# apache/tez

Hardware: NVIDIA H100
Metric: sorted KV GB/s (16B key / 64B val) (higher is better)
Workload: dtype u8

## Files before the change

### tez_b200/csrc/emit_fast.cuh

```cuda
#pragma once
#include "sorter_kernels.cuh"

#ifndef TEZGPU_EMIT_MIN_CTAS
#define TEZGPU_EMIT_MIN_CTAS 4
#endif

namespace tezgpu {

constexpr int FE_THREADS = 256;
constexpr int FE_MAX_RECS = 256;
constexpr int FE_IMG_BYTES = 22016;

struct TileDesc {
  uint32_t p;
  uint32_t r0;
  uint32_t nr;
  uint32_t flags;
  uint64_t abs0;
  uint64_t after;
};

struct TileCrc {
  uint32_t raw;
  uint32_t p;
// ... 6 lines not shown
  int lo = 0, hi = e.P;
  while (hi - lo > 1) {
    int mid = (lo + hi) >> 1;
    if (e.tile_start[mid] <= tile) lo = mid; else hi = mid;
  }
  const uint32_t p = (uint32_t)lo;
  const uint32_t ps = e.part_start[p], pe = e.part_start[p + 1];
  const uint32_t k = tile - e.tile_start[p];
  TileDesc d;
  d.p = p;
  d.r0 = ps + k * e.recs_per_tile;
  d.nr = min(e.recs_per_tile, pe - d.r0);
  const bool first = (k == 0), last = (d.r0 + d.nr == pe);
  d.flags = (first ? 1u : 0u) | (last ? 2u : 0u);
  const uint64_t seg0 = e.seg_start[p];
  d.abs0 = seg0 + (first ? 0 : 4 + (uint64_t)(d.r0 - ps) * e.rec_size);
  const uint64_t tile_end = seg0 + 4 + (uint64_t)(d.r0 - ps + d.nr) * e.rec_size + (last ? 2 : 0);
  d.after = (e.seg_start[p + 1] - 4) - tile_end;
  tiles[tile] = d;
}

__global__ void k_crc_combine(const TileCrc *__restrict__ tc, uint32_t ntiles, const CrcTables *__restrict__ t,
                              uint32_t *__restrict__ seg_crc) {
  uint32_t i = blockIdx.x * blockDim.x + threadIdx.x;
  const int lane = threadIdx.x & 31;
  uint32_t p = 0xFFFFFFFFu, val = 0;
  if (i < ntiles) {
    TileCrc c = tc[i];
    p = c.p;
    val = c.raw ? crc_shift_bytes(t, c.raw, c.after) : 0u;
  }
#pragma unroll
  for (int o = 1; o < 32; o <<= 1) {
    uint32_t v2 = __shfl_up_sync(0xffffffffu, val, o), p2 = __shfl_up_sync(0xffffffffu, p, o);
    if (lane >= o && p2 == p) val ^= v2;
  }
  uint32_t pn = __shfl_down_sync(0xffffffffu, p, 1);
  if (p != 0xFFFFFFFFu && (lane == 31 || pn != p) && val) atomicXor(&seg_crc[p], val);
}

__device__ __forceinline__ void sts_b8(uint32_t a, uint32_t v) { asm volatile("st.shared.b8 [%0], %1;" ::"r"(a), "r"(v) : "memory"); }
__device__ __forceinline__ void sts_b16(uint32_t a, uint32_t v) { asm volatile("st.shared.b16 [%0], %1;" ::"r"(a), "h"((unsigned short)v) : "memory"); }
__device__ __forceinline__ void sts_b32(uint32_t a, uint32_t v) { asm volatile("st.shared.b32 [%0], %1;" ::"r"(a), "r"(v) : "memory"); }
__device__ __forceinline__ void sts_v4(uint32_t a, uint4 v) {
  asm volatile("st.shared.v4.b32 [%0], {%1,%2,%3,%4};" ::"r"(a), "r"(v.x), "r"(v.y), "r"(v.z), "r"(v.w) : "memory");
}

__device__ __forceinline__ void sts16_unaligned(uint32_t a, uint4 v) {
  const uint32_t al = a & 3u;
  if (al == 0) {
    if ((a & 15u) == 0) sts_v4(a, v);
    else { sts_b32(a, v.x); sts_b32(a + 4, v.y); sts_b32(a + 8, v.z); sts_b32(a + 12, v.w); }
  } else if (al == 2) {
    sts_b16(a, v.x & 0xFFFFu);
    sts_b32(a + 2, __funnelshift_r(v.x, v.y, 16));
    sts_b32(a + 6, __funnelshift_r(v.y, v.z, 16));
    sts_b32(a + 10, __funnelshift_r(v.z, v.w, 16));
    sts_b16(a + 14, v.w >> 16);
  } else if (al == 1) {
    sts_b8(a, v.x & 0xFFu);
    sts_b16(a + 1, (v.x >> 8) & 0xFFFFu);
    sts_b32(a + 3, __funnelshift_r(v.x, v.y, 24));
    sts_b32(a + 7, __funnelshift_r(v.y, v.z, 24));
    sts_b32(a + 11, __funnelshift_r(v.z, v.w, 24));
    sts_b8(a + 15, v.w >> 24);
  } else {
    sts_b8(a, v.x & 0xFFu);
    sts_b32(a + 1, __funnelshift_r(v.x, v.y, 8));
    sts_b32(a + 5, __funnelshift_r(v.y, v.z, 8));
    sts_b32(a + 9, __funnelshift_r(v.z, v.w, 8));
    sts_b16(a + 13, (v.w >> 8) & 0xFFFFu);
    sts_b8(a + 15, v.w >> 24);
  }
}

__device__ __forceinline__ uint4 ldg_stream_v4(const void *p) {
  uint4 r;
  asm volatile("ld.global.nc.L1::no_allocate.v4.u32 {%0,%1,%2,%3}, [%4];"
               : "=r"(r.x), "=r"(r.y), "=r"(r.z), "=r"(r.w) : "l"(p));
  return r;
}
__device__ __forceinline__ void stg_stream_v4(void *p, uint4 v) {
  asm volatile("st.global.L1::no_allocate.v4.u32 [%0], {%1,%2,%3,%4};" ::"l"(p), "r"(v.x), "r"(v.y), "r"(v.z), "r"(v.w) : "memory");
}

struct FastEmitParams {
  EmitParams e;
  const TileDesc *tiles;
  TileCrc *tile_crc;
  uint32_t ntiles;
  uint32_t cpr;
  uint32_t cpr_magic;
  uint32_t stride;
};

__device__ __forceinline__ uint64_t fast_source_offset(const Records &rec, uint32_t ri, uint32_t stride, uint32_t p) {
  if (rec.use_runs) return run_record_off_p(rec.runs, p, ri) + rec.runs.hdr_len;
  return rec.key_off ? rec.key_off[ri] : (uint64_t)ri * stride;
}

template <int UNROLL, bool ALIGNED>
__global__ void __launch_bounds__(FE_THREADS, TEZGPU_EMIT_MIN_CTAS) k_emit_fast(FastEmitParams fp) {
  __shared__ __align__(16) uint8_t s_img[FE_IMG_BYTES];
  __shared__ uint32_t s_idx[2][FE_MAX_RECS];
  __shared__ uint64_t s_off[ALIGNED ? 1 : 2][ALIGNED ? 1 : FE_MAX_RECS];
  __shared__ uint32_t s_tab[4 * 256];
  __shared__ uint32_t s_adv32[4 * 256];
  __shared__ uint32_t s_part[FE_THREADS];

  const EmitParams &e = fp.e;
  const int tid = threadIdx.x, lane = tid & 31, warp = tid >> 5;
  for (int i = tid; i < 4 * 256; i += FE_THREADS) {
    s_tab[i] = (&e.crc->slice[0][0])[i];
    s_adv32[i] = (&e.crc->adv128[0][0])[i];
  }
  const uint32_t lane_pow = e.crc->pow_word[4 * (31 - lane)];
  WarpLinearMap m_word, m_skip;
  {
    const uint32_t *gt = &e.crc->slice[0][0], *ga = &e.crc->advc[0][0];
    m_word.init([&](uint32_t x) { return gt[768 + (x & 0xFF)] ^ gt[512 + ((x >> 8) & 0xFF)] ^ gt[256 + ((x >> 16) & 0xFF)] ^ gt[x >> 24]; }, lane);
    m_skip.init([&](uint32_t x) { return ga[x & 0xFF] ^ ga[256 + ((x >> 8) & 0xFF)] ^ ga[512 + ((x >> 16) & 0xFF)] ^ ga[768 + (x >> 24)]; }, lane);
  }
  const uint32_t img_base = (uint32_t)__cvta_generic_to_shared(s_img);
  const uint8_t *__restrict__ kv = e.rec.kv;
  const uint8_t *kv_end = kv + e.rec.kv_bytes;
  const uint32_t rec_size = e.rec_size, hdr_len = e.fixed_hdr_len, stride = fp.stride;

  TileDesc td_next;
  if (blockIdx.x < fp.ntiles) {
    td_next = fp.tiles[blockIdx.x];
    if ((uint32_t)tid < td_next.nr) {
      const uint32_t ri = e.order[td_next.r0 + tid];
      s_idx[0][tid] = ri;
      if (!ALIGNED) s_off[0][tid] = fast_source_offset(e.rec, ri, stride, td_next.p);
    }
  }
  uint32_t buf = 0;
  for (uint32_t tile = blockIdx.x; tile < fp.ntiles; tile += gridDim.x, buf ^= 1u) {
    const TileDesc td = td_next;
    const uint32_t nr = td.nr;
    const bool first_tile = td.flags & 1u, last_tile = td.flags & 2u;
    const uint32_t tile_n = tile + gridDim.x;
    if (tile_n < fp.ntiles) td_next = fp.tiles[tile_n];
    __syncthreads();
    const uint32_t *__restrict__ c_idx = s_idx[buf];
    const uint64_t *__restrict__ c_off = s_off[ALIGNED ? 0 : buf];
    const uint64_t abs0 = td.abs0;
    const uint32_t lead = (uint32_t)(abs0 & 15u);
    const uint32_t rec0 = lead + (first_tile ? 4u : 0u);
    const uint32_t body_end = rec0 + nr * rec_size + (last_tile ? 2u : 0u);

    const uint32_t npieces = nr * fp.cpr;
    const uint32_t half_up = (nr + 1) >> 1;
    for (uint32_t q0 = tid; q0 < npieces; q0 += FE_THREADS * UNROLL) {
      uint4 v[UNROLL];
      uint32_t dst[UNROLL];
#pragma unroll
      for (int u = 0; u < UNROLL; u++) {
        uint32_t q = q0 + u * FE_THREADS;
        if (q < npieces) {
          uint32_t jp = fp.cpr == 1 ? q : __umulhi(q, fp.cpr_magic);
          uint32_t c = q - jp * fp.cpr;
          uint32_t j = jp < half_up ? 2u * jp : 2u * (jp - half_up) + 1u;
          if (ALIGNED) {
            v[u] = ldg_stream_v4(kv + (uint64_t)c_idx[j] * stride + 16u * c);
          } else {
// ... 112 lines not shown
```

### tez_b200/csrc/emit_pipe.cuh

```cuda
#pragma once
#include "emit_fast.cuh"

#ifndef TEZGPU_EMIT4_MIN_CTAS
#define TEZGPU_EMIT4_MIN_CTAS 3
#endif

namespace tezgpu {

constexpr int FE4_BATCH = FE_THREADS / 32;
constexpr int FE4_UNROLL = 5;
constexpr int FE4_RUN = 5;
constexpr uint32_t FE4_RUN_BYTES = 16u * FE4_RUN;
constexpr int FE4_IMG_BYTES = FE_THREADS * FE4_RUN * 16;
constexpr int FE4_GROUPS = 2;
constexpr int FE4_PARKED = 4;
constexpr int FE4_WBITS = 7;
constexpr int FE4_WDIGITS = (32 + FE4_WBITS - 1) / FE4_WBITS;
constexpr int FE4_WENTRIES = ((FE4_WDIGITS - 1) << FE4_WBITS) + (1 << (32 - FE4_WBITS * (FE4_WDIGITS - 1)));

static inline uint32_t emit4_max_recs(uint32_t rec_size) {
  return std::min<uint32_t>(FE_MAX_RECS, (FE4_IMG_BYTES - 15 - 4 - 2) / rec_size);
}

constexpr uint32_t FE4_MAX_CPR = 8;

static inline bool emit4_fits(uint32_t recs, uint32_t cpr, uint32_t rec_size) {
  if (cpr > FE4_MAX_CPR || recs > emit4_max_recs(rec_size)) return false;
  return (uint64_t)recs * cpr <= (uint64_t)FE4_UNROLL * FE_THREADS;
}

__host__ __device__ __forceinline__ uint32_t emit4_wtab_value(const CrcTables *__restrict__ t, uint32_t k, uint32_t e) {
  const uint32_t v = e << (FE4_WBITS * k);
  return t->slice[3][v & 0xFF] ^ t->slice[2][(v >> 8) & 0xFF] ^ t->slice[1][(v >> 16) & 0xFF] ^ t->slice[0][v >> 24];
}

__host__ __device__ __forceinline__ uint32_t emit4_next_word(const uint8_t *wt, uint32_t x) {
  uint32_t r = 0;
#pragma unroll
  for (int k = 0; k < FE4_WDIGITS; k++) {
    constexpr int E = 7;
    const int sh = FE4_WBITS * k - E;
    const uint32_t m = (k + 1 < FE4_WDIGITS ? (1u << FE4_WBITS) - 1 : (1u << (32 - FE4_WBITS * k)) - 1) << E;
    const uint32_t off = (sh >= 0 ? x >> sh : x << -sh) & m;
    r ^= *reinterpret_cast<const uint32_t *>(wt + off + ((size_t)k << (FE4_WBITS + E)));
  }
  return r;
}

struct FoldMeta {
  uint4 tail;
  uint32_t tile;
  uint32_t start;
  uint32_t end;
  uint32_t tiny;
};

__device__ __forceinline__ uint4 lds_v4(uint32_t a) {
  uint4 v;
  asm volatile("ld.shared.v4.b32 {%0,%1,%2,%3}, [%4];" : "=r"(v.x), "=r"(v.y), "=r"(v.z), "=r"(v.w) : "r"(a));
  return v;
}

struct Emit4Smem {
  static constexpr size_t WTAB = (size_t)FE4_WENTRIES * 32 * 4;
  static constexpr size_t SHARED = WTAB + 256 * 4 + 4 * 256 * 4;
  static constexpr size_t GROUP = FE4_IMG_BYTES + 3 * FE_MAX_RECS * 4 + (size_t)FE4_PARKED * FE_THREADS * 4 + (size_t)FE4_PARKED * sizeof(FoldMeta);
  static constexpr size_t TOTAL = SHARED + FE4_GROUPS * GROUP;
};

template <int UNROLL>
__global__ void __launch_bounds__(FE_THREADS * FE4_GROUPS, 1) k_emit_fast4(FastEmitParams fp) {
  using L = Emit4Smem;
  constexpr int BATCH = FE4_PARKED;
  extern __shared__ __align__(16) uint8_t smem4[];
  uint32_t *s_wtab = reinterpret_cast<uint32_t *>(smem4);
  uint32_t *s_tab = reinterpret_cast<uint32_t *>(smem4 + L::WTAB);
  uint32_t *s_hor = s_tab + 256;
  const int sub = threadIdx.x / FE_THREADS, tid = threadIdx.x % FE_THREADS, lane = tid & 31, warp = tid >> 5;
  uint8_t *gbase = smem4 + L::SHARED + (size_t)sub * L::GROUP;
  uint8_t *s_img = gbase;
  uint32_t(*s_idx)[FE_MAX_RECS] = reinterpret_cast<uint32_t(*)[FE_MAX_RECS]>(gbase + FE4_IMG_BYTES);
  uint32_t(*s_part)[FE_THREADS] = reinterpret_cast<uint32_t(*)[FE_THREADS]>(gbase + FE4_IMG_BYTES + 3 * FE_MAX_RECS * 4);
  FoldMeta *s_meta = reinterpret_cast<FoldMeta *>(gbase + FE4_IMG_BYTES + 3 * FE_MAX_RECS * 4 + (size_t)BATCH * FE_THREADS * 4);
  auto group_sync = [&]() { asm volatile("bar.sync %0, %1;" ::"r"(sub + 1), "r"(FE_THREADS) : "memory"); };

  const EmitParams &e = fp.e;
  const uint32_t G = gridDim.x * FE4_GROUPS, ntiles = fp.ntiles;
  uint32_t tile = blockIdx.x * FE4_GROUPS + sub;
  for (int i = threadIdx.x; i < FE4_WENTRIES * 32; i += FE_THREADS * FE4_GROUPS)
    s_wtab[i] = emit4_wtab_value(e.crc, (uint32_t)(i >> 5) >> FE4_WBITS, (uint32_t)(i >> 5) & ((1u << FE4_WBITS) - 1));
  for (int i = threadIdx.x; i < 256; i += FE_THREADS * FE4_GROUPS) s_tab[i] = e.crc->slice[0][i];
  {
    const uint32_t x_hor = e.crc->pow0[FE4_RUN_BYTES * 32];
    for (int i = threadIdx.x; i < 4 * 256; i += FE_THREADS * FE4_GROUPS) s_hor[i] = crc_multmodp((uint32_t)(i & 255) << (8 * (i >> 8)), x_hor);
  }
  __syncthreads();
  if (tile >= ntiles) return;
  const uint32_t lane_pow = e.crc->pow0[FE4_RUN_BYTES * (31 - lane)];
  const uint8_t *wt = reinterpret_cast<const uint8_t *>(s_wtab + lane);
  auto next_word = [&](uint32_t x) -> uint32_t { return emit4_next_word(wt, x); };
  const uint32_t img_base = (uint32_t)__cvta_generic_to_shared(s_img);
  const uint8_t *__restrict__ kv = e.rec.kv;
  const uint32_t rec_size = e.rec_size, hdr_len = e.fixed_hdr_len, stride = fp.stride, cpr = fp.cpr;
  const TileDesc *__restrict__ tiles = fp.tiles;

  auto piece = [&](int u, uint32_t nr, uint32_t &j, uint32_t &c) -> bool {
    const uint32_t q = tid + u * FE_THREADS;
    const uint32_t jp = cpr == 1 ? q : __umulhi(q, fp.cpr_magic);
    c = q - jp * cpr;
    const uint32_t half_up = (nr + 1) >> 1;
    j = jp < half_up ? 2u * jp : 2u * (jp - half_up) + 1u;
    return q < nr * cpr;
  };
  const uint32_t full_nr = e.recs_per_tile;
  uint32_t pk[UNROLL], onmask = 0;
#pragma unroll
  for (int u = 0; u < UNROLL; u++) {
    uint32_t j, c;
    const bool on = piece(u, full_nr, j, c);
    pk[u] = on ? (j | (16u * c) << 8 | (j * rec_size + hdr_len + 16u * c) << 15) : 0u;
    onmask |= on ? 1u << u : 0u;
  }
  uint4 v[UNROLL];
  auto issue_gather = [&](uint32_t nr, const uint32_t *idx) {
    const uint8_t *src[UNROLL];
    bool on[UNROLL];
    if (nr == full_nr) {
#pragma unroll
      for (int u = 0; u < UNROLL; u++) {
        on[u] = (onmask >> u) & 1u;
        src[u] = kv + (uint64_t)idx[pk[u] & 0xFFu] * stride + ((pk[u] >> 8) & 0x7Fu);
      }
    } else {
#pragma unroll
      for (int u = 0; u < UNROLL; u++) {
        uint32_t j, c;
        on[u] = piece(u, nr, j, c);
        src[u] = kv + (uint64_t)idx[on[u] ? j : 0u] * stride + 16u * c;
      }
    }
    if (UNROLL == 5) asm volatile("" : "+l"(src[0]), "+l"(src[1]), "+l"(src[2]), "+l"(src[3]), "+l"(src[UNROLL - 1]));
#pragma unroll
    for (int u = 0; u < UNROLL; u++)
      if (on[u]) v[u] = ldg_stream_v4(src[u]);
  };
  const uint32_t hdr16 = (uint32_t)e.fixed_hdr[0] | (uint32_t)e.fixed_hdr[1] << 8;

  uint32_t nr0, fl0, nr1 = 0, fl1 = 0, r0_2 = 0, nr2 = 0;
  uint64_t abs0, abs1 = 0;
  {
    const TileDesc t0 = tiles[tile];
    nr0 = t0.nr; fl0 = t0.flags; abs0 = t0.abs0;
    if ((uint32_t)tid < nr0) s_idx[0][tid] = e.order[t0.r0 + tid];
    if (tile + G < ntiles) {
      const TileDesc t1 = tiles[tile + G];
      nr1 = t1.nr; fl1 = t1.flags; abs1 = t1.abs0;
      if ((uint32_t)tid < nr1) s_idx[1][tid] = e.order[t1.r0 + tid];
    }
    if (tile + 2 * (uint64_t)G < ntiles) { r0_2 = tiles[tile + 2 * G].r0; nr2 = tiles[tile + 2 * G].nr; }
  }
  group_sync();
  issue_gather(nr0, s_idx[0]);

  uint32_t n_it = 0, slot = 0;
  for (;; tile += G, n_it++) {
    const bool has1 = tile + G < ntiles, has2 = tile + 2 * (uint64_t)G < ntiles, has3 = tile + 3 * (uint64_t)G < ntiles;
    const uint32_t nr = nr0;
    const bool first_tile = fl0 & 1u, last_tile = fl0 & 2u;
    const uint32_t lead = (uint32_t)(abs0 & 15u);
    const uint32_t rec0 = lead + (first_tile ? 4u : 0u);
    const uint32_t body_end = rec0 + nr * rec_size + (last_tile ? 2u : 0u);

    uint32_t r_idx = 0, r0_3 = 0, nr3 = 0, nr2n = 0, fl2n = 0;
    uint64_t abs2n = 0;
    if (has2) {
      if ((uint32_t)tid < nr2) r_idx = e.order[r0_2 + tid];
      const TileDesc *t2 = tiles + tile + 2 * (uint64_t)G;
      nr2n = t2->nr; fl2n = t2->flags; abs2n = t2->abs0;
    }
    if (has3) { const TileDesc *t3 = tiles + tile + 3 * (uint64_t)G; r0_3 = t3->r0; nr3 = t3->nr; }

    if (nr == full_nr) {
#pragma unroll
      for (int u = 0; u < UNROLL; u++)
        if ((onmask >> u) & 1u) sts16_unaligned(img_base + rec0 + (pk[u] >> 15), v[u]);
    } else {
#pragma unroll
      for (int u = 0; u < UNROLL; u++) {
        uint32_t j, c;
        if (piece(u, nr, j, c)) sts16_unaligned(img_base + rec0 + j * rec_size + hdr_len + 16u * c, v[u]);
      }
    }
    if ((uint32_t)tid < nr) {
      const uint32_t a = img_base + rec0 + tid * rec_size;
      if (hdr_len == 2 && !(a & 1u)) sts_b16(a, hdr16);
      else for (uint32_t b = 0; b < hdr_len; b++) sts_b8(a + b, e.fixed_hdr[b]);
    }
    if (tid == 0) {
      if (first_tile) { s_img[lead] = 'T'; s_img[lead + 1] = 'I'; s_img[lead + 2] = 'F'; s_img[lead + 3] = 0; }
      if (last_tile) { s_img[body_end - 2] = 0xFF; s_img[body_end - 1] = 0xFF; }
    }
    group_sync();

    if (has1) issue_gather(nr1, s_idx[(n_it + 1) % 3]);

    const uint32_t cb0 = rec0, cb1 = body_end;
    const uint32_t ca = cb0 >> 4, cz = cb1 >> 4;
    uint8_t *dstg = e.out + (abs0 - lead);
    uint32_t c = 0;
    if (cz > ca) {
      const int32_t Cn = (int32_t)(cz - ca);
      for (int32_t i = tid; i < Cn; i += FE_THREADS) {
        const uint4 w = lds_v4(img_base + 16u * (ca + (uint32_t)i));
        if (i > 0 || 16u * ca >= lead) stg_stream_v4(dstg + 16u * (ca + (uint32_t)i), w);
        else for (uint32_t x = lead; x < 16u * ca + 16u; x++) dstg[x] = s_img[x];
      }
      const int32_t i0 = Cn - FE4_RUN * (FE_THREADS - tid);
#pragma unroll
      for (int k = 0; k < FE4_RUN; k++) {
        const int32_t i = i0 + k;
        if (i < 0) continue;
        uint4 w = lds_v4(img_base + 16u * (ca + (uint32_t)i));
        if (i == 0) {
          const uint32_t skip = cb0 & 15u;
          uint32_t ww[4] = {w.x, w.y, w.z, w.w};
#pragma unroll
          for (uint32_t q = 0; q < 4; q++) {
            if (skip >= 4 * q + 4) ww[q] = 0;
            else if (skip > 4 * q) ww[q] &= 0xFFFFFFFFu << (8u * (skip - 4 * q));
          }
          w = make_uint4(ww[0], ww[1], ww[2], ww[3]);
        }
        c = next_word(c ^ w.x);
        c = next_word(c ^ w.y);
        c = next_word(c ^ w.z);
        c = next_word(c ^ w.w);
      }
    }
    s_part[slot][tid] = c;
    if (tid == 0) {
      for (uint32_t x = max(lead, 16u * cz); x < body_end; x++) dstg[x] = s_img[x];
      if (ca > (lead >> 4)) for (uint32_t x = lead; x < 16u * ca; x++) dstg[x] = s_img[x];
      FoldMeta m;
      m.tail = *reinterpret_cast<const uint4 *>(s_img + 16u * cz);
      m.tile = tile;
      m.tiny = cz > ca ? 0u : 1u;
      m.start = cz > ca ? 0u : (cb0 & 15u);
      m.end = cb1 & 15u;
      s_meta[slot] = m;
    }
    if (has2) s_idx[(n_it + 2) % 3][tid] = r_idx;
    slot++;
    group_sync();

    if (slot == (uint32_t)BATCH || !has1) {
      if ((uint32_t)warp < slot) {
        uint32_t q = 0;
#pragma unroll
        for (int k = 0; k < FE_THREADS / 32; k++) {
          q = s_hor[q & 0xFF] ^ s_hor[256 + ((q >> 8) & 0xFF)] ^ s_hor[512 + ((q >> 16) & 0xFF)] ^ s_hor[768 + (q >> 24)];
          q ^= s_part[warp][lane + 32 * k];
        }
        q = crc_multmodp(q, lane_pow);
#pragma unroll
        for (int o = 16; o > 0; o >>= 1) q ^= __shfl_xor_sync(0xffffffffu, q, o);
        if (lane == 0) {
          const FoldMeta m = s_meta[warp];
          const uint32_t tw[4] = {m.tail.x, m.tail.y, m.tail.z, m.tail.w};
          uint32_t raw = m.tiny ? 0u : q;
          for (uint32_t b = m.start; b < m.end; b++) {
            const uint32_t byte = (tw[b >> 2] >> (8u * (b & 3u))) & 0xFFu;
            raw = s_tab[(raw ^ byte) & 0xFF] ^ (raw >> 8);
          }
          const TileDesc td = tiles[m.tile];
          TileCrc tc;
          tc.raw = raw;
          tc.p = td.p;
          tc.after = td.after;
          fp.tile_crc[m.tile] = tc;
        }
      }
      slot = 0;
    }
    if (!has1) break;
    asm volatile("" : "+r"(nr2n), "+r"(fl2n), "+l"(abs2n), "+r"(r0_3), "+r"(nr3));
    nr0 = nr1; fl0 = fl1; abs0 = abs1;
    nr1 = nr2n; fl1 = fl2n; abs1 = abs2n;
    r0_2 = r0_3; nr2 = nr3;
  }
}

}
```

### tez_b200/csrc/sorter.cuh

```cuda
#pragma once
#include <stddef.h>
#include <stdlib.h>
#include <string.h>

#include <vector>

#include "../../include/tezgpu.h"
#include "device_util.h"
#include "combine.cuh"
#include "emit_pipe_u.cuh"
#include "sorter_kernels.cuh"

namespace tezgpu {

__global__ void k_store_to_host(uint32_t *__restrict__ dst0, const uint32_t *__restrict__ src0, uint32_t n0, uint32_t *__restrict__ dst1,
                                const uint32_t *__restrict__ src1, uint32_t n1, uint32_t *__restrict__ dst2,
                                const uint32_t *__restrict__ src2, uint32_t n2) {
  for (uint32_t i = threadIdx.x; i < n0; i += blockDim.x) dst0[i] = src0[i];
  for (uint32_t i = threadIdx.x; i < n1; i += blockDim.x) dst1[i] = src1[i];
  for (uint32_t i = threadIdx.x; i < n2; i += blockDim.x) dst2[i] = src2[i];
  __threadfence_system();
}
static inline void store_to_host(cudaStream_t st, void *d0, const void *s0, size_t b0, void *d1 = nullptr, const void *s1 = nullptr,
                                 size_t b1 = 0, void *d2 = nullptr, const void *s2 = nullptr, size_t b2 = 0) {
// ... 10 lines not shown

struct DeviceConstants {
  CrcTables *d_crc = nullptr;
  static DeviceConstants &get(int device) {
    static DeviceConstants inst[64];
    DeviceConstants &d = inst[device & 63];
    if (!d.d_crc) {
      CrcTables *h = new CrcTables();
      crc_build_tables(*h, EMIT_CRC_STRIDE_WORDS);
      TG_CUDA(cudaMalloc((void **)&d.d_crc, sizeof(CrcTables)));
      TG_CUDA(cudaMemcpy(d.d_crc, h, sizeof(CrcTables), cudaMemcpyHostToDevice));
      delete h;
    }
    return d;
  }
};

constexpr uint32_t FRAMING_MAX_LEN = 10;
struct FixedFraming {
  uint8_t bytes[FRAMING_MAX_LEN];
  uint32_t len;
  uint32_t rec_size;
  uint64_t packed(uint32_t word = 0) const {
    uint64_t x = 0;
    for (uint32_t b = 8 * word; b < len && b < 8 * word + 8; b++) x |= (uint64_t)bytes[b] << (8 * (b - 8 * word));
    return x;
  }
};
static inline FixedFraming fixed_framing(uint32_t klen, uint32_t vlen) {
  FixedFraming f{};
  for (int b = 0; b < vint_size_u32(klen); b++) f.bytes[f.len++] = vint_byte_u32(klen, b);
  for (int b = 0; b < vint_size_u32(vlen); b++) f.bytes[f.len++] = vint_byte_u32(vlen, b);
  f.rec_size = f.len + klen + vlen;
  return f;
}

struct FramingMismatch {};

struct SortVerdict {
  int error;
  union { uint32_t large_groups; uint32_t batch_count; };
  unsigned long long dups;
  uint64_t totals[2];
};
struct SortScratch {
  uint32_t hist[8 * RADIX];
  uint32_t trivial[8];
  uint32_t tile_counter[8];
  SortVerdict verdict;
  uint32_t unused[2];
  unsigned long long ties;
};
constexpr size_t SORT_SCRATCH_BYTES = 16 * 1024;
struct SortHostScratch {
  SortVerdict verdict;
  uint32_t ties;
  uint64_t total;
  uint32_t trivial[8];
  static constexpr size_t INDEX_OFFSET = 4096;
  int64_t *index() { return reinterpret_cast<int64_t *>(reinterpret_cast<uint8_t *>(this) + INDEX_OFFSET); }
};
static_assert(offsetof(SortScratch, trivial) == 2048 * 4 && offsetof(SortScratch, tile_counter) == 2056 * 4 &&
                  offsetof(SortScratch, verdict) == 2064 * 4 && sizeof(SortVerdict) == 32 && offsetof(SortScratch, ties) == 2074 * 4 &&
                  sizeof(SortScratch) <= SORT_SCRATCH_BYTES && offsetof(SortHostScratch, ties) == 32 &&
                  sizeof(SortHostScratch) <= SortHostScratch::INDEX_OFFSET, "sort scratch layout");

enum class FixedEmitKernel {
  Pipe,
  Fast,
  PipeUnaligned,
  FastUnaligned,
  General,
};
struct FixedEmitPlan {
  FixedEmitKernel kernel;
  uint32_t recs_per_tile;
};

static inline FixedEmitPlan plan_fixed_emit(const Records &rec, uint32_t rec_size) {
  const uint32_t stride = rec.klen + rec.vlen, cpr = stride / 16;
  const uint32_t cap = std::max<uint32_t>(1, std::min<uint32_t>(EMIT_MAX_RECS, (FE_IMG_BYTES - 32) / rec_size));
  if (stride < 16 || stride % 16 || (uint64_t)rec_size + 15 + 4 + 2 > FE_IMG_BYTES) return {FixedEmitKernel::General, cap};
  if (!rec.key_off && !rec.use_runs && ((uintptr_t)rec.kv & 15u) == 0) {
    const uint32_t m = emit4_max_recs(rec_size);
    if (emit4_fits(m, cpr, rec_size)) return {FixedEmitKernel::Pipe, std::min(cap, m)};
    return {FixedEmitKernel::Fast, cap};
  }
  const uint32_t m = emit4u_max_recs(cpr);
  if (m == 0) return {FixedEmitKernel::FastUnaligned, cap};
  const uint32_t top = std::min(cap, m);
  uint32_t best = top;
  double best_eff = 0;
  for (uint32_t r = top; r >= top - top / 10; r--) {
    const uint64_t chunks = ((uint64_t)r * rec_size + 15 + 4 + 2 + 15) / 16;
    const uint64_t rounds = (chunks + FE_THREADS - 1) / FE_THREADS;
    const double eff = (double)r / (double)rounds;
    if (eff > best_eff) { best_eff = eff; best = r; }
  }
  return {FixedEmitKernel::PipeUnaligned, best};
}

class SortPipeline {
 public:
  tezgpu_conf conf;
  int pbits;
  cudaStream_t stream = nullptr;
  EventTimer timer;
  int num_sms = 132;

  DeviceBuffer sortA, sortB, same, blk, small, tile_state, sizes, rec_off;
  DeviceBuffer t_pos[2], t_gid[2], t_lidx[2], t_key64[2], t_val[2], t_state, t_ghead, t_gneq, sym_sets, sym_tab, rep_flags;
  DeviceBuffer seg_start, tile_start, part_start, d_index, seg_crc, tile_desc, tile_crc, tie_state;
  PinnedBuffer h_small;

  explicit SortPipeline(const tezgpu_conf &c) : conf(c) {
    TG_CHECK(c.num_partitions >= 1, TEZGPU_E_INVALID, "num_partitions must be >= 1");
    TG_CHECK(c.comparator >= TEZGPU_CMP_BYTES && c.comparator <= TEZGPU_CMP_LONG, TEZGPU_E_UNSUPPORTED,
             "comparator outside the device-supported set (BYTES, TEXT, BYTESWRITABLE, INT, LONG)");
    TG_CHECK(c.partitioner == TEZGPU_PART_GIVEN || c.partitioner == TEZGPU_PART_HASH || c.partitioner == TEZGPU_PART_TOTAL_ORDER,
             TEZGPU_E_UNSUPPORTED, "partitioner outside the device-supported set (GIVEN, HASH, TOTAL_ORDER)");
    int ndev = 0;
    cudaError_t e = cudaGetDeviceCount(&ndev);
    if (e != cudaSuccess || ndev == 0) {
      cudaGetLastError();
      throw Error(TEZGPU_E_CUDA, "no CUDA device available (libtezgpu has no CPU fallback)");
    }
    TG_CHECK(c.device >= 0 && c.device < ndev, TEZGPU_E_INVALID, "bad device ordinal");
    TG_CUDA(cudaSetDevice(c.device));
    TG_CUDA(cudaStreamCreateWithFlags(&stream, cudaStreamNonBlocking));
    TG_CUDA(cudaDeviceGetAttribute(&num_sms, cudaDevAttrMultiProcessorCount, c.device));
    {
      const char *g = getenv("TEZGPU_L2_FETCH");
      int gran = g ? atoi(g) : 32;
      if (gran > 0 && cudaDeviceSetLimit(cudaLimitMaxL2FetchGranularity, (size_t)gran) != cudaSuccess) cudaGetLastError();
    }
    pbits = partition_bits(c.num_partitions);
    TG_CHECK(pbits <= 31, TEZGPU_E_INVALID, "too many partitions");
    h_small.ensure(SortHostScratch::INDEX_OFFSET);
    small.ensure(SORT_SCRATCH_BYTES);
    DeviceConstants::get(c.device);
  }
  ~SortPipeline() {
    if (stream) cudaStreamDestroy(stream);
  }

  static uint64_t output_bound(uint64_t n, uint64_t kv_bytes, int P) { return kv_bytes + 12 * n + 10ull * P + 64; }

  SortScratch *d_scratch() const { return small.as<SortScratch>(); }
  SortHostScratch *h_scratch() const { return h_small.as<SortHostScratch>(); }

  struct SortState {
    Records rec;
    uint32_t *K = nullptr;
    uint32_t *order = nullptr;
    uint64_t dup_count = 0, tie_records = 0;
    int launches = 0;
    bool have_bounds = false, spec_layout = false;
    const uint8_t *same = nullptr;
  } state;
  int merge_check_same = 1;
  bool merge_inputs_plain = false;
  int combiner = TEZGPU_COMBINE_NONE;
  DeviceBuffer sp_prefix, sp_len, sp_off, sp_blob;
  SplitTable splits{};
  bool have_splits = false;
  void set_split_points(const HostSplitTable &t) {
    TG_CUDA(cudaSetDevice(conf.device));
    const size_t n = t.prefix.size();
// ... 311 lines not shown
  void emit_phase(int rle, bool merge_mode, uint8_t *d_out, uint64_t out_cap, uint64_t *out_len, int64_t *index,
                  tezgpu_stats *stats) {
    TG_CUDA(cudaSetDevice(conf.device));
    TG_CHECK(((uintptr_t)d_out & 15u) == 0, TEZGPU_E_INVALID, "output buffer must be 16-byte aligned");
    const Records rec = state.rec;
    const uint32_t n = rec.n;
    const int P = conf.num_partitions;
    uint32_t *K = state.K, *order = state.order;
    const uint64_t dup_count = state.dup_count, tie_records = state.tie_records;
    int launches = state.launches;
    const CrcTables *d_crc = DeviceConstants::get(conf.device).d_crc;
    const size_t n4 = (size_t)(n ? n : 1) * 4;
    TG_CUDA(cudaMemsetAsync(seg_crc.p, 0, (size_t)P * 4, stream));
    if (timer.n > (n ? 4 : 2)) timer.n = n ? 4 : 2;

    EmitParams e = make_emit_params(rec, order, rle, merge_mode, d_out);
    if (!state.have_bounds) {
      k_part_bounds<<<(uint32_t)div_up((uint64_t)P + 1, 256), 256, 0, stream>>>(K, n, P, pbits, part_start.as<uint32_t>());
      launches++;
    }
    const bool no_repeats = !rle && (!merge_mode || (!merge_check_same && merge_inputs_plain));
    const bool fixed_emit = rec.fixed && (dup_count == 0 || no_repeats);
    uint64_t bound = output_bound(n, rec.fixed ? (uint64_t)n * (rec.klen + rec.vlen) : rec.kv_bytes, P);
    const FixedEmitKernel kernel = fixed_emit ? set_fixed_layout(e, rec) : FixedEmitKernel::General;
    if (!fixed_emit || !state.spec_layout) {
      if (!fixed_emit) {
        uint64_t avg = n ? (rec.fixed ? (uint64_t)(rec.klen + rec.vlen) : rec.kv_bytes / n) + 4 : 16;
        e.recs_per_tile = (uint32_t)std::max<uint64_t>(1, std::min<uint64_t>(EMIT_MAX_RECS, (EMIT_IMG_BYTES - 32) / avg));
        sizes.ensure(n4);
        rec_off.ensure(((size_t)n + 2) * 8);
        if (n) {
          rep_flags.ensure(n);
          k_emit_repeat_flags<<<(uint32_t)div_up(n, 256), 256, 0, stream>>>(e, K, rep_flags.as<uint8_t>());
          launches++;
          e.rep = rep_flags.as<uint8_t>();
          k_emit_sizes<<<(uint32_t)div_up(n, 256), 256, 0, stream>>>(e, K, sizes.as<uint32_t>());
          launches += 1 + scan_u32_exclusive(stream, blk, sizes.as<uint32_t>(), n, rec_off.as<uint64_t>());
          TG_CUDA(cudaGetLastError());
        } else {
          TG_CUDA(cudaMemsetAsync(rec_off.p, 0, 16, stream));
        }
        e.rec_off = rec_off.as<uint64_t>();
      }
      k_layout<<<1, 1024, 0, stream>>>(e, seg_start.as<uint64_t>(), tile_start.as<uint32_t>(), d_index.as<int64_t>(), d_scratch()->verdict.totals);
      launches++;
      TG_CUDA(cudaGetLastError());
      store_to_host(stream, h_scratch()->verdict.totals, d_scratch()->verdict.totals, 16, h_scratch()->index(), d_index.p, (size_t)P * 24);
      TG_CUDA(cudaGetLastError());
      TG_CUDA(cudaStreamSynchronize(stream));
      state.spec_layout = false;
    }
    const uint64_t file_bytes = h_scratch()->verdict.totals[0];
    const uint64_t tiles = h_scratch()->verdict.totals[1];
    TG_CHECK(file_bytes <= bound, TEZGPU_E_INVALID, "internal: output exceeds bound");
    TG_CHECK(file_bytes <= out_cap, TEZGPU_E_NOMEM, "output buffer too small for file.out");
    const bool source_oriented = fixed_emit && kernel != FixedEmitKernel::General;
    const uint32_t stride = rec.klen + rec.vlen;
    FastEmitParams fp;
    if (tiles && source_oriented) {
      tile_desc.ensure((size_t)tiles * sizeof(TileDesc));
      k_build_tiles<<<(uint32_t)div_up(tiles, 256), 256, 0, stream>>>(e, tile_desc.as<TileDesc>());
      launches++;
      fp.e = e;
      tile_crc.ensure((size_t)tiles * sizeof(TileCrc));
      fp.tile_crc = tile_crc.as<TileCrc>();
      fp.tiles = tile_desc.as<TileDesc>();
      fp.ntiles = (uint32_t)tiles;
      fp.cpr = stride / 16;
      fp.cpr_magic = fp.cpr == 1 ? 0u : (uint32_t)((1ull << 32) / fp.cpr) + 1u;
      fp.stride = stride;
    }
    timer.mark(stream);
    if (tiles) {
      auto persistent_grid = [&](auto kern, int threads, size_t smem) {
        int per_sm = 0;
        TG_CUDA(cudaOccupancyMaxActiveBlocksPerMultiprocessor(&per_sm, kern, threads, smem));
        return (uint32_t)std::min<uint64_t>(tiles, (uint64_t)num_sms * (per_sm > 0 ? per_sm : 1));
      };
      if (!fixed_emit) {
        k_emit<false><<<persistent_grid(k_emit<false>, EMIT_THREADS, 0), EMIT_THREADS, 0, stream>>>(e);
      } else {
        switch (kernel) {
          case FixedEmitKernel::Pipe: {
            set_smem_limit<k_emit_fast4<FE4_UNROLL>>(conf.device, Emit4Smem::TOTAL);
            const uint32_t grid = (uint32_t)std::min<uint64_t>(div_up(tiles, FE4_GROUPS), (uint64_t)num_sms);
            k_emit_fast4<FE4_UNROLL><<<grid, FE_THREADS * FE4_GROUPS, Emit4Smem::TOTAL, stream>>>(fp);
            break;
          }
          case FixedEmitKernel::Fast:
            k_emit_fast<5, true><<<persistent_grid(k_emit_fast<5, true>, FE_THREADS, 0), FE_THREADS, 0, stream>>>(fp);
            break;
          case FixedEmitKernel::PipeUnaligned:
            set_smem_limit<k_emit_fast4u<FE4U_UNROLL>>(conf.device, Emit4uSmem::TOTAL);
            k_emit_fast4u<FE4U_UNROLL><<<persistent_grid(k_emit_fast4u<FE4U_UNROLL>, FE_THREADS, Emit4uSmem::TOTAL), FE_THREADS,
                                         Emit4uSmem::TOTAL, stream>>>(fp);
            break;
          case FixedEmitKernel::FastUnaligned:
            k_emit_fast<5, false><<<persistent_grid(k_emit_fast<5, false>, FE_THREADS, 0), FE_THREADS, 0, stream>>>(fp);
            break;
          case FixedEmitKernel::General:
            k_emit<true><<<persistent_grid(k_emit<true>, EMIT_THREADS, 0), EMIT_THREADS, 0, stream>>>(e);
            break;
        }
      }
      if (source_oriented) {
        k_crc_combine<<<(uint32_t)div_up(tiles, 256), 256, 0, stream>>>(fp.tile_crc, (uint32_t)tiles, d_crc, seg_crc.as<uint32_t>());
        launches++;
      }
      launches++;
      TG_CUDA(cudaGetLastError());
    }
    timer.mark(stream);
    k_finalize_segments<<<(uint32_t)div_up(P, 256), 256, 0, stream>>>(e);
    launches++;
    TG_CUDA(cudaGetLastError());
    timer.mark(stream);
    TG_CUDA(cudaStreamSynchronize(stream));

    if (out_len) *out_len = file_bytes;
    const int64_t *hidx = h_scratch()->index();
    if (index) memcpy(index, hidx, (size_t)P * 24);
    if (stats) {
      memset(stats, 0, sizeof(*stats));
      stats->output_records = n;
      int64_t raw = 0;
      for (int p = 0; p < P; p++) raw += hidx[3 * p + 1];
      stats->output_bytes_with_overhead = raw;
      stats->output_bytes_physical = (int64_t)file_bytes;
      stats->file_out_bytes = (int64_t)file_bytes;
      stats->spilled_records = n;
      stats->num_spills = 1;
      stats->rle_used = rle;
      stats->adjacent_equal_keys = (int64_t)dup_count;
      stats->tie_records = (int64_t)tie_records;
      const int b = n ? 3 : 1;
      stats->ms_stage = n ? timer.ms(0, 1) : 0;
      stats->ms_sort = n ? timer.ms(1, 2) : 0;
      stats->ms_ties = n ? timer.ms(2, 3) : 0;
      stats->ms_emit = timer.ms(b, b + 3);
      stats->ms_emit_kernel = timer.ms(b + 1, b + 2);
      stats->ms_total = timer.ms(0, b + 3);
      stats->kernel_launches = launches;
    }
  }

  bool combine_phase() {
    const Records rec = state.rec;
    const uint32_t n = rec.n, W = combine_width(combiner);
    TG_CHECK(W, TEZGPU_E_INVALID, "unknown combiner");
    const char *name = combiner == TEZGPU_COMBINE_SUM_INT ? "IntSumReducer needs 4-byte IntWritable values"
                                                          : "LongSumReducer needs 8-byte LongWritable values";
    if (n == 0) return false;
    c_bad.ensure(16);
    c_host.ensure(64);
    uint32_t *bad = c_bad.as<uint32_t>();
    TG_CUDA(cudaMemsetAsync(bad, 0xFF, 4, stream));
    int launches = 0;
    if (state.dup_count == 0) {
      if (rec.fixed) {
        TG_CHECK(rec.vlen == W, TEZGPU_E_INVALID, "combiner: record 0 has a " + std::to_string(rec.vlen) + "-byte value (" + name + ")");
        return false;
      }
      k_combine_check_width<<<(uint32_t)std::min<uint64_t>(div_up(n, 256), (uint64_t)num_sms * 16), 256, 0, stream>>>(rec, W, bad);
      TG_CUDA(cudaGetLastError());
      state.launches += 1;
      uint32_t *h = c_host.as<uint32_t>();
      TG_CUDA(cudaMemcpyAsync(h, bad, 4, cudaMemcpyDeviceToHost, stream));
      TG_CUDA(cudaStreamSynchronize(stream));
      TG_CHECK(h[0] == 0xFFFFFFFFu, TEZGPU_E_INVALID, "combiner: record " + std::to_string(h[0]) + " has a value of the wrong width (" + name + ")");
// ... 118 lines not shown
```

Before: 532.8.

## Feed emit kernel via warp-specialized bulk-copy producers and mbarrier ring

```diff
diff --git a/tez_b200/csrc/emit_fast.cuh b/tez_b200/csrc/emit_fast.cuh
--- a/tez_b200/csrc/emit_fast.cuh
+++ b/tez_b200/csrc/emit_fast.cuh
@@ -112,6 +112,31 @@
 }
 __device__ __forceinline__ void stg_stream_v4(void *p, uint4 v) {
   asm volatile("st.global.L1::no_allocate.v4.u32 [%0], {%1,%2,%3,%4};" ::"l"(p), "r"(v.x), "r"(v.y), "r"(v.z), "r"(v.w) : "memory");
+}
+
+__device__ __forceinline__ void mbar_init(uint32_t bar, uint32_t count) {
+  asm volatile("mbarrier.init.shared::cta.b64 [%0], %1;" ::"r"(bar), "r"(count) : "memory");
+}
+__device__ __forceinline__ void mbar_expect_tx(uint32_t bar, uint32_t bytes) {
+  asm volatile("mbarrier.arrive.expect_tx.shared::cta.b64 _, [%0], %1;" ::"r"(bar), "r"(bytes) : "memory");
+}
+__device__ __forceinline__ void mbar_arrive(uint32_t bar) {
+  asm volatile("mbarrier.arrive.shared::cta.b64 _, [%0];" ::"r"(bar) : "memory");
+}
+__device__ __forceinline__ void mbar_wait(uint32_t bar, uint32_t parity) {
+  asm volatile(
+      "{\n"
+      ".reg .pred p;\n"
+      "WAIT_%=:\n"
+      "mbarrier.try_wait.parity.shared::cta.b64 p, [%0], %1;\n"
+      "@p bra DONE_%=;\n"
+      "bra WAIT_%=;\n"
+      "DONE_%=:\n"
+      "}\n" ::"r"(bar), "r"(parity) : "memory");
+}
+__device__ __forceinline__ void bulk_g2s(uint32_t dst, const void *src, uint32_t bytes, uint32_t bar) {
+  asm volatile("cp.async.bulk.shared::cluster.global.mbarrier::complete_tx::bytes [%0], [%1], %2, [%3];" ::"r"(dst), "l"(src),
+               "r"(bytes), "r"(bar) : "memory");
 }
 
 struct FastEmitParams {
diff --git a/tez_b200/csrc/emit_pipe.cuh b/tez_b200/csrc/emit_pipe.cuh
--- a/tez_b200/csrc/emit_pipe.cuh
+++ b/tez_b200/csrc/emit_pipe.cuh
@@ -8,12 +8,14 @@
 namespace tezgpu {
 
 constexpr int FE4_BATCH = FE_THREADS / 32;
-constexpr int FE4_UNROLL = 5;
 constexpr int FE4_RUN = 5;
 constexpr uint32_t FE4_RUN_BYTES = 16u * FE4_RUN;
 constexpr int FE4_IMG_BYTES = FE_THREADS * FE4_RUN * 16;
 constexpr int FE4_GROUPS = 2;
 constexpr int FE4_PARKED = 4;
+constexpr int FE4_PRODUCERS = 4;
+constexpr int FE4_STAGES = 4;
+constexpr int FE4_CTA_THREADS = FE_THREADS * FE4_GROUPS + 32 * FE4_PRODUCERS;
 constexpr int FE4_WBITS = 7;
 constexpr int FE4_WDIGITS = (32 + FE4_WBITS - 1) / FE4_WBITS;
 constexpr int FE4_WENTRIES = ((FE4_WDIGITS - 1) << FE4_WBITS) + (1 << (32 - FE4_WBITS * (FE4_WDIGITS - 1)));
@@ -23,11 +25,6 @@
 }
 
 constexpr uint32_t FE4_MAX_CPR = 8;
-
-static inline bool emit4_fits(uint32_t recs, uint32_t cpr, uint32_t rec_size) {
-  if (cpr > FE4_MAX_CPR || recs > emit4_max_recs(rec_size)) return false;
-  return (uint64_t)recs * cpr <= (uint64_t)FE4_UNROLL * FE_THREADS;
-}
 
 __host__ __device__ __forceinline__ uint32_t emit4_wtab_value(const CrcTables *__restrict__ t, uint32_t k, uint32_t e) {
   const uint32_t v = e << (FE4_WBITS * k);
@@ -64,46 +61,102 @@
 struct Emit4Smem {
   static constexpr size_t WTAB = (size_t)FE4_WENTRIES * 32 * 4;
   static constexpr size_t SHARED = WTAB + 256 * 4 + 4 * 256 * 4;
-  static constexpr size_t GROUP = FE4_IMG_BYTES + 3 * FE_MAX_RECS * 4 + (size_t)FE4_PARKED * FE_THREADS * 4 + (size_t)FE4_PARKED * sizeof(FoldMeta);
-  static constexpr size_t TOTAL = SHARED + FE4_GROUPS * GROUP;
+  static constexpr size_t GROUP = FE4_IMG_BYTES + (size_t)FE4_PARKED * FE_THREADS * 4 + (size_t)FE4_PARKED * sizeof(FoldMeta);
+  static constexpr size_t BARS = SHARED + FE4_GROUPS * GROUP;
+  static constexpr size_t RING = BARS + 2 * FE4_STAGES * 8;
+  static constexpr size_t TOTAL = RING + (size_t)FE4_STAGES * FE4_IMG_BYTES;
+  static_assert(RING % 16 == 0 && FE4_STAGES % FE4_GROUPS == 0, "Emit4Smem layout");
 };
 
-template <int UNROLL>
-__global__ void __launch_bounds__(FE_THREADS * FE4_GROUPS, 1) k_emit_fast4(FastEmitParams fp) {
+template <int STAGES>
+__global__ void __launch_bounds__(FE4_CTA_THREADS, 1) k_emit_fast4(FastEmitParams fp) {
   using L = Emit4Smem;
   constexpr int BATCH = FE4_PARKED;
   extern __shared__ __align__(16) uint8_t smem4[];
   uint32_t *s_wtab = reinterpret_cast<uint32_t *>(smem4);
   uint32_t *s_tab = reinterpret_cast<uint32_t *>(smem4 + L::WTAB);
   uint32_t *s_hor = s_tab + 256;
+  const uint32_t full0 = (uint32_t)__cvta_generic_to_shared(smem4 + L::BARS), empty0 = full0 + 8 * STAGES;
+  const uint32_t ring0 = (uint32_t)__cvta_generic_to_shared(smem4 + L::RING);
+
+  const EmitParams &e = fp.e;
+  const uint32_t G = gridDim.x * FE4_GROUPS, ntiles = fp.ntiles;
+  for (int i = threadIdx.x; i < FE4_WENTRIES * 32; i += FE4_CTA_THREADS)
+    s_wtab[i] = emit4_wtab_value(e.crc, (uint32_t)(i >> 5) >> FE4_WBITS, (uint32_t)(i >> 5) & ((1u << FE4_WBITS) - 1));
+  for (int i = threadIdx.x; i < 256; i += FE4_CTA_THREADS) s_tab[i] = e.crc->slice[0][i];
+  {
+    const uint32_t x_hor = e.crc->pow0[FE4_RUN_BYTES * 32];
+    for (int i = threadIdx.x; i < 4 * 256; i += FE4_CTA_THREADS) s_hor[i] = crc_multmodp((uint32_t)(i & 255) << (8 * (i >> 8)), x_hor);
+  }
+  if (threadIdx.x == 0) {
+    for (int s = 0; s < STAGES; s++) {
+      mbar_init(full0 + 8 * s, FE4_PRODUCERS);
+      mbar_init(empty0 + 8 * s, 1);
+    }
+    asm volatile("fence.mbarrier_init.release.cluster;" ::: "memory");
+  }
+  __syncthreads();
+  const uint8_t *__restrict__ kv = e.rec.kv;
+  const uint32_t rec_size = e.rec_size, hdr_len = e.fixed_hdr_len, stride = fp.stride;
+  const TileDesc *__restrict__ tiles = fp.tiles;
+
+  if (threadIdx.x >= FE_THREADS * FE4_GROUPS) {
+    constexpr int RPL = FE_MAX_RECS / (32 * FE4_PRODUCERS);
+    const uint32_t pw = (threadIdx.x - FE_THREADS * FE4_GROUPS) >> 5, lane = threadIdx.x & 31;
+    auto tile_of = [&](uint32_t n) -> uint64_t {
+      return (uint64_t)blockIdx.x * FE4_GROUPS + n % FE4_GROUPS + (uint64_t)(n / FE4_GROUPS) * G;
+    };
+    auto rec_of = [&](int k) -> uint32_t { return 32u * (pw + FE4_PRODUCERS * (uint32_t)k) + lane; };
+    if (tile_of(0) >= ntiles) return;
+    uint32_t nr = tiles[tile_of(0)].nr, nr1 = 0, r0_1 = 0;
+    uint32_t idx[RPL];
+    {
+      const uint32_t r0 = tiles[tile_of(0)].r0;
+#pragma unroll
+      for (int k = 0; k < RPL; k++) idx[k] = rec_of(k) < nr ? e.order[r0 + rec_of(k)] : 0u;
+    }
+    if (tile_of(1) < ntiles) { nr1 = tiles[tile_of(1)].nr; r0_1 = tiles[tile_of(1)].r0; }
+    for (uint32_t n = 0;; n++) {
+      const bool has1 = tile_of(n + 1) < ntiles, has2 = tile_of(n + 2) < ntiles;
+      uint32_t nidx[RPL], nr2 = 0, r0_2 = 0;
+      if (has1) {
+#pragma unroll
+        for (int k = 0; k < RPL; k++) nidx[k] = rec_of(k) < nr1 ? e.order[r0_1 + rec_of(k)] : 0u;
+      }
+      if (has2) { const TileDesc *t2 = tiles + tile_of(n + 2); nr2 = t2->nr; r0_2 = t2->r0; }
+      const uint32_t s = n % STAGES, full = full0 + 8 * s;
+      if (n >= (uint32_t)STAGES) mbar_wait(empty0 + 8 * s, ((n / STAGES) & 1u) ^ 1u);
+      uint32_t mine = 0;
+#pragma unroll
+      for (int k = 0; k < RPL; k++) mine += rec_of(k) < nr ? 1u : 0u;
+      const uint32_t warp_recs = __reduce_add_sync(0xffffffffu, mine);
+      if (lane == 0) mbar_expect_tx(full, warp_recs * stride);
+      __syncwarp();
+      const uint32_t dst = ring0 + s * FE4_IMG_BYTES;
+#pragma unroll
+      for (int k = 0; k < RPL; k++)
+        if (rec_of(k) < nr) bulk_g2s(dst + rec_of(k) * stride, kv + (uint64_t)idx[k] * stride, stride, full);
+      if (!has1) break;
+#pragma unroll
+      for (int k = 0; k < RPL; k++) idx[k] = nidx[k];
+      nr = nr1; nr1 = nr2; r0_1 = r0_2;
+    }
+    return;
+  }
+
   const int sub = threadIdx.x / FE_THREADS, tid = threadIdx.x % FE_THREADS, lane = tid & 31, warp = tid >> 5;
   uint8_t *gbase = smem4 + L::SHARED + (size_t)sub * L::GROUP;
   uint8_t *s_img = gbase;
-  uint32_t(*s_idx)[FE_MAX_RECS] = reinterpret_cast<uint32_t(*)[FE_MAX_RECS]>(gbase + FE4_IMG_BYTES);
-  uint32_t(*s_part)[FE_THREADS] = reinterpret_cast<uint32_t(*)[FE_THREADS]>(gbase + FE4_IMG_BYTES + 3 * FE_MAX_RECS * 4);
-  FoldMeta *s_meta = reinterpret_cast<FoldMeta *>(gbase + FE4_IMG_BYTES + 3 * FE_MAX_RECS * 4 + (size_t)BATCH * FE_THREADS * 4);
+  uint32_t(*s_part)[FE_THREADS] = reinterpret_cast<uint32_t(*)[FE_THREADS]>(gbase + FE4_IMG_BYTES);
+  FoldMeta *s_meta = reinterpret_cast<FoldMeta *>(gbase + FE4_IMG_BYTES + (size_t)BATCH * FE_THREADS * 4);
   auto group_sync = [&]() { asm volatile("bar.sync %0, %1;" ::"r"(sub + 1), "r"(FE_THREADS) : "memory"); };
-
-  const EmitParams &e = fp.e;
-  const uint32_t G = gridDim.x * FE4_GROUPS, ntiles = fp.ntiles;
   uint32_t tile = blockIdx.x * FE4_GROUPS + sub;
-  for (int i = threadIdx.x; i < FE4_WENTRIES * 32; i += FE_THREADS * FE4_GROUPS)
-    s_wtab[i] = emit4_wtab_value(e.crc, (uint32_t)(i >> 5) >> FE4_WBITS, (uint32_t)(i >> 5) & ((1u << FE4_WBITS) - 1));
-  for (int i = threadIdx.x; i < 256; i += FE_THREADS * FE4_GROUPS) s_tab[i] = e.crc->slice[0][i];
-  {
-    const uint32_t x_hor = e.crc->pow0[FE4_RUN_BYTES * 32];
-    for (int i = threadIdx.x; i < 4 * 256; i += FE_THREADS * FE4_GROUPS) s_hor[i] = crc_multmodp((uint32_t)(i & 255) << (8 * (i >> 8)), x_hor);
-  }
-  __syncthreads();
   if (tile >= ntiles) return;
   const uint32_t lane_pow = e.crc->pow0[FE4_RUN_BYTES * (31 - lane)];
   const uint8_t *wt = reinterpret_cast<const uint8_t *>(s_wtab + lane);
   auto next_word = [&](uint32_t x) -> uint32_t { return emit4_next_word(wt, x); };
   const uint32_t img_base = (uint32_t)__cvta_generic_to_shared(s_img);
-  const uint8_t *__restrict__ kv = e.rec.kv;
-  const uint32_t rec_size = e.rec_size, hdr_len = e.fixed_hdr_len, stride = fp.stride, cpr = fp.cpr;
-  const TileDesc *__restrict__ tiles = fp.tiles;
-
+  const uint32_t cpr = fp.cpr;
   auto piece = [&](int u, uint32_t nr, uint32_t &j, uint32_t &c) -> bool {
     const uint32_t q = tid + u * FE_THREADS;
     const uint32_t jp = cpr == 1 ? q : __umulhi(q, fp.cpr_magic);
@@ -113,83 +166,55 @@
     return q < nr * cpr;
   };
   const uint32_t full_nr = e.recs_per_tile;
-  uint32_t pk[UNROLL], onmask = 0;
-#pragma unroll
-  for (int u = 0; u < UNROLL; u++) {
+  uint32_t pk[FE4_RUN], onmask = 0;
+#pragma unroll
+  for (int u = 0; u < FE4_RUN; u++) {
     uint32_t j, c;
     const bool on = piece(u, full_nr, j, c);
-    pk[u] = on ? (j | (16u * c) << 8 | (j * rec_size + hdr_len + 16u * c) << 15) : 0u;
+    pk[u] = on ? (j * stride + 16u * c) | (j * rec_size + hdr_len + 16u * c) << 15 : 0u;
     onmask |= on ? 1u << u : 0u;
   }
-  uint4 v[UNROLL];
-  auto issue_gather = [&](uint32_t nr, const uint32_t *idx) {
-    const uint8_t *src[UNROLL];
-    bool on[UNROLL];
-    if (nr == full_nr) {
-#pragma unroll
-      for (int u = 0; u < UNROLL; u++) {
-        on[u] = (onmask >> u) & 1u;
-        src[u] = kv + (uint64_t)idx[pk[u] & 0xFFu] * stride + ((pk[u] >> 8) & 0x7Fu);
-      }
-    } else {
-#pragma unroll
-      for (int u = 0; u < UNROLL; u++) {
-        uint32_t j, c;
-        on[u] = piece(u, nr, j, c);
-        src[u] = kv + (uint64_t)idx[on[u] ? j : 0u] * stride + 16u * c;
-      }
-    }
-    if (UNROLL == 5) asm volatile("" : "+l"(src[0]), "+l"(src[1]), "+l"(src[2]), "+l"(src[3]), "+l"(src[UNROLL - 1]));
-#pragma unroll
-    for (int u = 0; u < UNROLL; u++)
-      if (on[u]) v[u] = ldg_stream_v4(src[u]);
-  };
   const uint32_t hdr16 = (uint32_t)e.fixed_hdr[0] | (uint32_t)e.fixed_hdr[1] << 8;
 
-  uint32_t nr0, fl0, nr1 = 0, fl1 = 0, r0_2 = 0, nr2 = 0;
-  uint64_t abs0, abs1 = 0;
-  {
-    const TileDesc t0 = tiles[tile];
-    nr0 = t0.nr; fl0 = t0.flags; abs0 = t0.abs0;
-    if ((uint32_t)tid < nr0) s_idx[0][tid] = e.order[t0.r0 + tid];
-    if (tile + G < ntiles) {
-      const TileDesc t1 = tiles[tile + G];
-      nr1 = t1.nr; fl1 = t1.flags; abs1 = t1.abs0;
-      if ((uint32_t)tid < nr1) s_idx[1][tid] = e.order[t1.r0 + tid];
-    }
-    if (tile + 2 * (uint64_t)G < ntiles) { r0_2 = tiles[tile + 2 * G].r0; nr2 = tiles[tile + 2 * G].nr; }
-  }
-  group_sync();
-  issue_gather(nr0, s_idx[0]);
-
-  uint32_t n_it = 0, slot = 0;
-  for (;; tile += G, n_it++) {
-    const bool has1 = tile + G < ntiles, has2 = tile + 2 * (uint64_t)G < ntiles, has3 = tile + 3 * (uint64_t)G < ntiles;
-    const uint32_t nr = nr0;
-    const bool first_tile = fl0 & 1u, last_tile = fl0 & 2u;
+  TileDesc td = tiles[tile];
+  uint32_t slot = 0;
+  for (uint32_t n = sub;; tile += G, n += FE4_GROUPS) {
+    const bool has1 = tile + G < ntiles;
+    TileDesc td1;
+    if (has1) td1 = tiles[tile + G];
+    const uint32_t nr = td.nr;
+    const bool first_tile = td.flags & 1u, last_tile = td.flags & 2u;
+    const uint64_t abs0 = td.abs0;
     const uint32_t lead = (uint32_t)(abs0 & 15u);
     const uint32_t rec0 = lead + (first_tile ? 4u : 0u);
-    const uint32_t body_end = rec0 + nr * rec_size + (last_tile ? 2u : 0u);
-
-    uint32_t r_idx = 0, r0_3 = 0, nr3 = 0, nr2n = 0, fl2n = 0;
-    uint64_t abs2n = 0;
-    if (has2) {
-      if ((uint32_t)tid < nr2) r_idx = e.order[r0_2 + tid];
-      const TileDesc *t2 = tiles + tile + 2 * (uint64_t)G;
-      nr2n = t2->nr; fl2n = t2->flags; abs2n = t2->abs0;
-    }
-    if (has3) { const TileDesc *t3 = tiles + tile + 3 * (uint64_t)G; r0_3 = t3->r0; nr3 = t3->nr; }
-
-    if (nr == full_nr) {
-#pragma unroll
-      for (int u = 0; u < UNROLL; u++)
-        if ((onmask >> u) & 1u) sts16_unaligned(img_base + rec0 + (pk[u] >> 15), v[u]);
-    } else {
-#pragma unroll
-      for (int u = 0; u < UNROLL; u++) {
-        uint32_t j, c;
-        if (piece(u, nr, j, c)) sts16_unaligned(img_base + rec0 + j * rec_size + hdr_len + 16u * c, v[u]);
-      }
+    const uint32_t recs_end = rec0 + nr * rec_size;
+    const uint32_t body_end = recs_end + (last_tile ? 2u : 0u);
+
+    const uint32_t s = n % STAGES;
+    mbar_wait(full0 + 8 * s, (n / STAGES) & 1u);
+    const uint32_t ring = ring0 + s * FE4_IMG_BYTES;
+    {
+      uint4 v[FE4_RUN];
+      uint32_t dst[FE4_RUN];
+      bool on[FE4_RUN];
+#pragma unroll
+      for (int u = 0; u < FE4_RUN; u++) {
+        uint32_t src = 0;
+        if (nr == full_nr) {
+          on[u] = (onmask >> u) & 1u;
+          src = pk[u] & 0x7FFFu;
+          dst[u] = pk[u] >> 15;
+        } else {
+          uint32_t j, c;
+          on[u] = piece(u, nr, j, c);
+          src = j * stride + 16u * c;
+          dst[u] = j * rec_size + hdr_len + 16u * c;
+        }
+        if (on[u]) v[u] = lds_v4(ring + src);
+      }
+#pragma unroll
+      for (int u = 0; u < FE4_RUN; u++)
+        if (on[u]) sts16_unaligned(img_base + rec0 + dst[u], v[u]);
     }
     if ((uint32_t)tid < nr) {
       const uint32_t a = img_base + rec0 + tid * rec_size;
@@ -201,8 +226,7 @@
       if (last_tile) { s_img[body_end - 2] = 0xFF; s_img[body_end - 1] = 0xFF; }
     }
     group_sync();
-
-    if (has1) issue_gather(nr1, s_idx[(n_it + 1) % 3]);
+    if (tid == 0) mbar_arrive(empty0 + 8 * s);
 
     const uint32_t cb0 = rec0, cb1 = body_end;
     const uint32_t ca = cb0 >> 4, cz = cb1 >> 4;
@@ -249,7 +273,6 @@
       m.end = cb1 & 15u;
       s_meta[slot] = m;
     }
-    if (has2) s_idx[(n_it + 2) % 3][tid] = r_idx;
     slot++;
     group_sync();
 
@@ -272,22 +295,19 @@
             const uint32_t byte = (tw[b >> 2] >> (8u * (b & 3u))) & 0xFFu;
             raw = s_tab[(raw ^ byte) & 0xFF] ^ (raw >> 8);
           }
-          const TileDesc td = tiles[m.tile];
+          const TileDesc tdm = tiles[m.tile];
           TileCrc tc;
           tc.raw = raw;
-          tc.p = td.p;
-          tc.after = td.after;
+          tc.p = tdm.p;
+          tc.after = tdm.after;
           fp.tile_crc[m.tile] = tc;
         }
       }
       slot = 0;
     }
     if (!has1) break;
-    asm volatile("" : "+r"(nr2n), "+r"(fl2n), "+l"(abs2n), "+r"(r0_3), "+r"(nr3));
-    nr0 = nr1; fl0 = fl1; abs0 = abs1;
-    nr1 = nr2n; fl1 = fl2n; abs1 = abs2n;
-    r0_2 = r0_3; nr2 = nr3;
-  }
-}
-
-}
+    td = td1;
+  }
+}
+
+}
diff --git a/tez_b200/csrc/sorter.cuh b/tez_b200/csrc/sorter.cuh
--- a/tez_b200/csrc/sorter.cuh
+++ b/tez_b200/csrc/sorter.cuh
@@ -116,8 +116,7 @@
   const uint32_t cap = std::max<uint32_t>(1, std::min<uint32_t>(EMIT_MAX_RECS, (FE_IMG_BYTES - 32) / rec_size));
   if (stride < 16 || stride % 16 || (uint64_t)rec_size + 15 + 4 + 2 > FE_IMG_BYTES) return {FixedEmitKernel::General, cap};
   if (!rec.key_off && !rec.use_runs && ((uintptr_t)rec.kv & 15u) == 0) {
-    const uint32_t m = emit4_max_recs(rec_size);
-    if (emit4_fits(m, cpr, rec_size)) return {FixedEmitKernel::Pipe, std::min(cap, m)};
+    if (cpr <= FE4_MAX_CPR) return {FixedEmitKernel::Pipe, std::min(cap, emit4_max_recs(rec_size))};
     return {FixedEmitKernel::Fast, cap};
   }
   const uint32_t m = emit4u_max_recs(cpr);
@@ -595,9 +594,9 @@
       } else {
         switch (kernel) {
           case FixedEmitKernel::Pipe: {
-            set_smem_limit<k_emit_fast4<FE4_UNROLL>>(conf.device, Emit4Smem::TOTAL);
+            set_smem_limit<k_emit_fast4<FE4_STAGES>>(conf.device, Emit4Smem::TOTAL);
             const uint32_t grid = (uint32_t)std::min<uint64_t>(div_up(tiles, FE4_GROUPS), (uint64_t)num_sms);
-            k_emit_fast4<FE4_UNROLL><<<grid, FE_THREADS * FE4_GROUPS, Emit4Smem::TOTAL, stream>>>(fp);
+            k_emit_fast4<FE4_STAGES><<<grid, FE4_CTA_THREADS, Emit4Smem::TOTAL, stream>>>(fp);
             break;
           }
           case FixedEmitKernel::Fast:
```

Result: faster. 552.6, median of 6 (+3.7%).
